# shiveshkhaitan/novel_view_synthesis_3d

Measured on NVIDIA B200. Metric: xunet_train_images_per_sec, higher is better.
Workload: dtype bf16

## Files before the change

novel_view_synthesis_3d_b200/csrc/attn_tc.cu:

```cuda
#include "kernels.h"
#include "tc_common.cuh"

namespace {

struct AttnTcParams {
  const bf16* res;
  bf16* out;
  float* lse;
  int L, C, heads, cross;
  float scale_log2;
  float* cstats;
};

constexpr int kQT = 128;
constexpr int kKB = 64;

__host__ __device__ constexpr int fwd_kv_stages(int hd) { return hd <= 32 ? 6 : 3; }
template <int HD>
__global__ void __launch_bounds__(192) attn_fwd_tc_kernel(const __grid_constant__ CUtensorMap tmQ128,
                                                          const __grid_constant__ CUtensorMap tmKV64, const AttnTcParams p) {
  constexpr int CW = HD < 64 ? HD : 64;
  constexpr int NCH = HD / CW;
  constexpr int TILE = 128 * CW * 2;
  constexpr int TILE_B = kKB * CW * 2;
  constexpr int KV_STAGES = fwd_kv_stages(HD);
  constexpr int P_BYTES = 128 * kKB * 2;
  constexpr int S_BUFS = 2;
  constexpr uint32_t TMEM_COLS = 256;
  constexpr int O_COL = S_BUFS * kKB;
  extern __shared__ uint8_t smem_raw[];
  uint8_t* base = reinterpret_cast<uint8_t*>((reinterpret_cast<uintptr_t>(smem_raw) + 1023) & ~(uintptr_t)1023);
  uint8_t* smQ = base;
  uint8_t* smK = smQ + NCH * TILE;
  uint8_t* smV = smK + KV_STAGES * NCH * TILE_B;
  uint8_t* smP = smV + KV_STAGES * NCH * TILE_B;
  uint64_t* bars = reinterpret_cast<uint64_t*>(smP + 2 * P_BYTES);
  uint64_t* q_full = bars;
  uint64_t* kv_full = bars + 1;
  uint64_t* kv_empty = kv_full + KV_STAGES;
  uint64_t* s_full = kv_empty + KV_STAGES;
  uint64_t* p_full = s_full + 2;
  uint64_t* o_full = p_full + 2;
  uint64_t* o_free = o_full + 1;
  uint32_t* tmem_slot = reinterpret_cast<uint32_t*>(o_free + 1);

  const int warp = threadIdx.x >> 5, lane = threadIdx.x & 31;
  const int q0 = blockIdx.x * kQT, h = blockIdx.y, n = blockIdx.z;
  const int nkv = p.cross ? (n ^ 1) : n;
  const int nkb = p.L / kKB;

  if (threadIdx.x == 0) {
    mbar_init(q_full, 1);
    for (int s = 0; s < KV_STAGES; ++s) { mbar_init(&kv_full[s], 1); mbar_init(&kv_empty[s], 1); }
    for (int s = 0; s < 2; ++s) { mbar_init(&s_full[s], 1); mbar_init(&p_full[s], 128); }
    mbar_init(o_full, 1);
    mbar_init(o_free, 128);
    asm volatile("fence.mbarrier_init.release.cluster;" ::: "memory");
    asm volatile("prefetch.tensormap [%0];" ::"l"(&tmQ128) : "memory");
    asm volatile("prefetch.tensormap [%0];" ::"l"(&tmKV64) : "memory");
  }
  if (warp == 1) tmem_alloc(tmem_slot, TMEM_COLS);
  tcgen05_fence_before();
  __syncthreads();
  tcgen05_fence_after();
  xu_grid_dep_sync();
  const uint32_t tmem_base = *tmem_slot;
  const uint32_t tmem_O = tmem_base + O_COL;

  if (warp == 0) {
    if (lane == 0) {
      mbar_expect_tx(q_full, NCH * TILE);
      for (int c = 0; c < NCH; ++c) tma_load_3d(smQ + c * TILE, &tmQ128, q_full, h * HD + c * CW, q0, n);
      for (int j = 0; j < nkb; ++j) {
        const int s = j % KV_STAGES;
        mbar_wait(&kv_empty[s], ((j / KV_STAGES) & 1) ^ 1);
        mbar_expect_tx(&kv_full[s], 2 * NCH * TILE_B);
        for (int c = 0; c < NCH; ++c) {
          tma_load_3d(smK + (s * NCH + c) * TILE_B, &tmKV64, &kv_full[s], p.C + h * HD + c * CW, j * kKB, nkv);
          tma_load_3d(smV + (s * NCH + c) * TILE_B, &tmKV64, &kv_full[s], 2 * p.C + h * HD + c * CW, j * kKB, nkv);
        }
      }
    }
  } else if (warp == 1) {
    if (lane == 0) {
      const uint32_t idesc_s = make_idesc_bf16(kKB, 0, 0);
      const uint32_t idesc_o = make_idesc_bf16(HD, 0, 1);
      auto issue_s = [&](int j) {
        const int s = j % KV_STAGES;
        mbar_wait(&kv_full[s], (j / KV_STAGES) & 1);
        tcgen05_fence_after();
#pragma unroll
        for (int c = 0; c < NCH; ++c)
#pragma unroll
          for (int k = 0; k < CW / 16; ++k)
            umma_bf16(tmem_base + (j % S_BUFS) * kKB, make_kmajor_desc<CW>(smem_u32(smQ + c * TILE) + k * 32),
                      make_kmajor_desc<CW>(smem_u32(smK + (s * NCH + c) * TILE_B) + k * 32), idesc_s, (c > 0 || k > 0) ? 1u : 0u);
        umma_commit(&s_full[j & 1]);
      };
      mbar_wait(q_full, 0);
      issue_s(0);
      for (int j = 0; j < nkb; ++j) {
        const int s = j % KV_STAGES;
        if (S_BUFS == 2 && j + 1 < nkb) issue_s(j + 1);
        mbar_wait(&p_full[j & 1], (j >> 1) & 1);
        if (S_BUFS == 1 && j + 1 < nkb) issue_s(j + 1);
        if (j > 0) mbar_wait(o_free, (j - 1) & 1);
        tcgen05_fence_after();
#pragma unroll
        for (int kk = 0; kk < kKB / 16; ++kk) {
          const uint64_t dp = make_kmajor_desc<64>(smem_u32(smP + (j & 1) * P_BYTES) + kk * 32);
          const uint64_t dv = make_mnmajor_desc<CW>(smem_u32(smV + s * NCH * TILE_B) + kk * 16 * (CW * 2), TILE_B);
          umma_bf16(tmem_O, dp, dv, idesc_o, kk > 0 ? 1u : 0u);
        }
        umma_commit(o_full);
        umma_commit(&kv_empty[s]);
      }
    }
  } else {
    const int lane_base = (warp & 3) * 32;
    const int r = lane_base + lane;
    const uint32_t lane_addr = (uint32_t)lane_base << 16;
    float m = -INFINITY, l = 0.f, corr_prev = 0.f;
    float acc[HD];
#pragma unroll
    for (int i = 0; i < HD; ++i) acc[i] = 0.f;
    const uint32_t prow_off = (r >> 3) * 1024 + (r & 7) * 128;
    auto absorb_o = [&](int jj, float corr) {
      mbar_wait(o_full, jj & 1);
      tcgen05_fence_after();
#pragma unroll
      for (int c0 = 0; c0 < HD; c0 += 16) {
        uint32_t v[16];
        asm volatile(
            "tcgen05.ld.sync.aligned.32x32b.x16.b32 {%0, %1, %2, %3, %4, %5, %6, %7, %8, %9, %10, %11, %12, %13, %14, %15}, [%16];"
            : "=r"(v[0]), "=r"(v[1]), "=r"(v[2]), "=r"(v[3]), "=r"(v[4]), "=r"(v[5]), "=r"(v[6]), "=r"(v[7]), "=r"(v[8]),
              "=r"(v[9]), "=r"(v[10]), "=r"(v[11]), "=r"(v[12]), "=r"(v[13]), "=r"(v[14]), "=r"(v[15])
            : "r"(tmem_O + lane_addr + c0));
        asm volatile("tcgen05.wait::ld.sync.aligned;" ::: "memory");
#pragma unroll
        for (int i = 0; i < 16; ++i) acc[c0 + i] = fmaf(acc[c0 + i], corr, __uint_as_float(v[i]));
      }
      tcgen05_fence_before();
      mbar_arrive(o_free);
    };
    for (int j = 0; j < nkb; ++j) {
      mbar_wait(&s_full[j & 1], (j >> 1) & 1);
      tcgen05_fence_after();
      uint32_t v[2][32];
      tmem_ld32_nowait(tmem_base + (j % S_BUFS) * kKB + lane_addr, v[0]);
      tmem_ld32_nowait(tmem_base + (j % S_BUFS) * kKB + lane_addr + 32, v[1]);
      asm volatile("tcgen05.wait::ld.sync.aligned;" ::: "memory");
      float mq[4] = {-INFINITY, -INFINITY, -INFINITY, -INFINITY};
#pragma unroll
      for (int i = 0; i < 32; i += 4)
#pragma unroll
        for (int c = 0; c < 4; ++c) mq[c] = fmaxf(mq[c], fmaxf(__uint_as_float(v[0][i + c]), __uint_as_float(v[1][i + c])));
      const float mraw = fmaxf(fmaxf(mq[0], mq[1]), fmaxf(mq[2], mq[3]));
      const float mx = fmaxf(m, mraw * p.scale_log2);
      const float corr = ex2_approx(m - mx);
      float rsq[4] = {0.f, 0.f, 0.f, 0.f};
      uint8_t* prow = smP + (j & 1) * P_BYTES + prow_off;
#pragma unroll
      for (int hh = 0; hh < 2; ++hh)
#pragma unroll
        for (int g = 0; g < 4; ++g) {
          uint4 pk;
          uint32_t* pw = reinterpret_cast<uint32_t*>(&pk);
#pragma unroll
          for (int q = 0; q < 4; ++q) {
            const float p0 = ex2_approx(fmaf(__uint_as_float(v[hh][g * 8 + 2 * q]), p.scale_log2, -mx));
            const float p1 = ex2_approx(fmaf(__uint_as_float(v[hh][g * 8 + 2 * q + 1]), p.scale_log2, -mx));
            rsq[q] += p0 + p1;
            __nv_bfloat162 b2 = __floats2bfloat162_rn(p0, p1);
            pw[q] = *reinterpret_cast<uint32_t*>(&b2);
          }
          const int chunk = hh * 4 + g;
          sts128(prow + ((chunk ^ (r & 7)) << 4), pk);
        }
      l = l * corr + ((rsq[0] + rsq[1]) + (rsq[2] + rsq[3]));
      m = mx;
      fence_async_smem();
      tcgen05_fence_before();
      mbar_arrive(&p_full[j & 1]);
      if (j > 0) absorb_o(j - 1, corr_prev);
      corr_prev = corr;
    }
    absorb_o(nkb - 1, corr_prev);
    const float inv = 1.f / l;
    const long long o = ((long long)n * p.L + q0 + r) * p.C + h * HD;
    float* cs_row = p.cstats ? p.cstats + ((long long)(n >> 1) * p.C + h * HD) * 2 : nullptr;
    float sx[32];
#pragma unroll
    for (int c0 = 0; c0 < HD; c0 += 8) {
      uint4 rv = *reinterpret_cast<const uint4*>(p.res + o + c0);
      const __nv_bfloat162* r2 = reinterpret_cast<const __nv_bfloat162*>(&rv);
      uint4 ov;
// ... 32 lines not shown
};

constexpr int kBB = 64;

__device__ __forceinline__ void bulk_load_1d(void* dst, const void* src, uint32_t bytes, uint64_t* bar) {
  asm volatile("cp.async.bulk.shared::cluster.global.mbarrier::complete_tx::bytes [%0], [%1], %2, [%3];" ::"r"(smem_u32(dst)),
               "l"(src), "r"(bytes), "r"(smem_u32(bar))
               : "memory");
}
__device__ __forceinline__ void tmem_ld16(uint32_t taddr, uint32_t (&v)[16]) {
  asm volatile(
      "tcgen05.ld.sync.aligned.32x32b.x16.b32 {%0, %1, %2, %3, %4, %5, %6, %7, %8, %9, %10, %11, %12, %13, %14, %15}, [%16];"
      : "=r"(v[0]), "=r"(v[1]), "=r"(v[2]), "=r"(v[3]), "=r"(v[4]), "=r"(v[5]), "=r"(v[6]), "=r"(v[7]), "=r"(v[8]), "=r"(v[9]),
        "=r"(v[10]), "=r"(v[11]), "=r"(v[12]), "=r"(v[13]), "=r"(v[14]), "=r"(v[15])
      : "r"(taddr));
  asm volatile("tcgen05.wait::ld.sync.aligned;" ::: "memory");
}

__device__ __forceinline__ void tmem_ld8(uint32_t taddr, uint32_t (&v)[8]) {
  asm volatile("tcgen05.ld.sync.aligned.32x32b.x8.b32 {%0, %1, %2, %3, %4, %5, %6, %7}, [%8];"
               : "=r"(v[0]), "=r"(v[1]), "=r"(v[2]), "=r"(v[3]), "=r"(v[4]), "=r"(v[5]), "=r"(v[6]), "=r"(v[7])
               : "r"(taddr));
  asm volatile("tcgen05.wait::ld.sync.aligned;" ::: "memory");
}

template <int HD>
__global__ void __launch_bounds__(320) attn_bwd_dq_tc_kernel(const __grid_constant__ CUtensorMap tmQ128,
                                                             const __grid_constant__ CUtensorMap tmQ64,
                                                             const __grid_constant__ CUtensorMap tmG128,
                                                             const AttnBwdParams p) {
  constexpr int CW = HD < 64 ? HD : 64;
  constexpr int NCH = HD / CW;
  constexpr int TILE = 128 * CW * 2;
  constexpr int TILE_B = kBB * CW * 2;
  constexpr int STAGES = 2;
  constexpr uint32_t TMEM_COLS = (2 * kBB + HD) <= 256 ? 256 : 512;
  extern __shared__ uint8_t smem_raw[];
// ... 337 lines not shown
#pragma unroll
      for (int q = 0; q < 8; ++q) a2[q] = __floats2bfloat162_rn(__uint_as_float(a[2 * q]) * sc, __uint_as_float(a[2 * q + 1]) * sc);
      *reinterpret_cast<uint4*>(dst + cc) = oa[0];
      *reinterpret_cast<uint4*>(dst + cc + 8) = oa[1];
    }
  }
  tcgen05_fence_before();
  __syncthreads();
  if (warp == 1) {
    tcgen05_fence_after();
    tmem_dealloc(tmem_base, TMEM_COLS);
  }
}

__host__ __device__ constexpr int fused_stages(int hd) { return hd <= 16 ? 4 : 3; }
template <int HD>
__global__ void __launch_bounds__(320, 2) attn_bwd_fused_tc_kernel(const __grid_constant__ CUtensorMap tmQ128,
                                                              const __grid_constant__ CUtensorMap tmQ64,
                                                              const __grid_constant__ CUtensorMap tmG64,
                                                              const __grid_constant__ CUtensorMap tmO64,
                                                              const __grid_constant__ CUtensorMap tmR64,
                                                              const AttnBwdParams p) {
  constexpr int CW = HD < 64 ? HD : 64;
  constexpr int NCH = HD / CW;
  constexpr int TILE = 128 * CW * 2;
  constexpr int TILE_B = kBB * CW * 2;
  constexpr int STAGES = fused_stages(HD);
  constexpr uint32_t TMEM_COLS = 256;
  static_assert(2 * kBB + 4 * HD <= 256, "fused backward: head_dim <= 32");
  extern __shared__ uint8_t smem_raw[];
  uint8_t* base = reinterpret_cast<uint8_t*>((reinterpret_cast<uintptr_t>(smem_raw) + 1023) & ~(uintptr_t)1023);
  uint8_t* smK = base;
  uint8_t* smV = smK + NCH * TILE;
  uint8_t* smQ = smV + NCH * TILE;
  uint8_t* smG = smQ + STAGES * NCH * TILE_B;
  uint8_t* smPT = smG + STAGES * NCH * TILE_B;
  float* smL = reinterpret_cast<float*>(smPT + 2 * 32768);
  float* smD = smL + STAGES * kBB;
  float* smW = smD + STAGES * kBB;
  uint8_t* smO = reinterpret_cast<uint8_t*>(smW + 8 * 64);
  uint8_t* smR = smO + (p.fold ? STAGES * NCH * TILE_B : 0);
  uint64_t* bars = reinterpret_cast<uint64_t*>(smR + (p.fold ? STAGES * NCH * TILE_B : 0));
  uint64_t* kv_full = bars;
  uint64_t* q_full = bars + 1;
  uint64_t* q_empty = q_full + STAGES;
  uint64_t* sp_full = q_empty + STAGES;
  uint64_t* pt_full = sp_full + 1;
  uint64_t* dkv_full = pt_full + 1;
  uint64_t* s_free = dkv_full + 1;
  uint64_t* pt_empty = s_free + 1;
  uint32_t* tmem_slot = reinterpret_cast<uint32_t*>(pt_empty + 2);

// ... 6 lines not shown
    for (int s = 0; s < STAGES; ++s) { mbar_init(&q_full[s], 1); mbar_init(&q_empty[s], 1); }
    mbar_init(sp_full, 1);
    mbar_init(pt_full, 256);
    mbar_init(dkv_full, 1);
    mbar_init(s_free, 256);
    mbar_init(&pt_empty[0], 1); mbar_init(&pt_empty[1], 1);
    asm volatile("fence.mbarrier_init.release.cluster;" ::: "memory");
  }
  if (warp == 1) tmem_alloc(tmem_slot, TMEM_COLS);
  tcgen05_fence_before();
  __syncthreads();
  tcgen05_fence_after();
  xu_grid_dep_sync();
  const uint32_t tmem_base = *tmem_slot;
  const uint32_t tmem_S = tmem_base, tmem_dP = tmem_base + kBB, tmem_dK = tmem_base + 2 * kBB, tmem_dV = tmem_dK + HD, tmem_dQ = tmem_dV + HD;
  const long long lrow = ((long long)nq * p.heads + h) * p.L;

  if (warp == 0) {
    if (lane == 0) {
      mbar_expect_tx(kv_full, 2 * NCH * TILE);
      for (int c = 0; c < NCH; ++c) {
        tma_load_3d(smK + c * TILE, &tmQ128, kv_full, p.C + h * HD + c * CW, k0, mfr);
        tma_load_3d(smV + c * TILE, &tmQ128, kv_full, 2 * p.C + h * HD + c * CW, k0, mfr);
      }
      for (int i = 0; i < nb; ++i) {
        const int s = i % STAGES;
        mbar_wait(&q_empty[s], ((i / STAGES) & 1) ^ 1);
        mbar_expect_tx(&q_full[s], p.fold ? 4 * NCH * TILE_B + kBB * 4 : 2 * NCH * TILE_B + 2 * kBB * 4);
        for (int c = 0; c < NCH; ++c) {
          tma_load_3d(smQ + (s * NCH + c) * TILE_B, &tmQ64, &q_full[s], h * HD + c * CW, i * kBB, nq);
          tma_load_3d(smG + (s * NCH + c) * TILE_B, &tmG64, &q_full[s], h * HD + c * CW, i * kBB, nq);
          if (p.fold) {
            tma_load_3d(smO + (s * NCH + c) * TILE_B, &tmO64, &q_full[s], h * HD + c * CW, i * kBB, nq);
            tma_load_3d(smR + (s * NCH + c) * TILE_B, &tmR64, &q_full[s], h * HD + c * CW, i * kBB, nq);
          }
        }
        bulk_load_1d(smL + s * kBB, p.lse + lrow + i * kBB, kBB * 4, &q_full[s]);
        if (!p.fold) bulk_load_1d(smD + s * kBB, p.Dbuf + lrow + i * kBB, kBB * 4, &q_full[s]);
      }
    }
  } else if (warp == 1) {
    if (lane == 0) {
      const uint32_t idesc_s = make_idesc_bf16(kBB, 0, 0);
      const uint32_t idesc_o = make_idesc_bf16(HD, 0, 1);
      const uint32_t idesc_dq = make_idesc_bf16(HD, 1, 1);
      mbar_wait(kv_full, 0);
      auto issue_scores = [&](int blk) {
        const int s = blk % STAGES;
        mbar_wait(&q_full[s], (blk / STAGES) & 1);
        tcgen05_fence_after();
#pragma unroll
        for (int c = 0; c < NCH; ++c)
#pragma unroll
          for (int k = 0; k < CW / 16; ++k) {
            const uint32_t acc = (c > 0 || k > 0) ? 1u : 0u;
            umma_bf16(tmem_S, make_kmajor_desc<CW>(smem_u32(smK + c * TILE) + k * 32),
                      make_kmajor_desc<CW>(smem_u32(smQ + (s * NCH + c) * TILE_B) + k * 32), idesc_s, acc);
            umma_bf16(tmem_dP, make_kmajor_desc<CW>(smem_u32(smV + c * TILE) + k * 32),
                      make_kmajor_desc<CW>(smem_u32(smG + (s * NCH + c) * TILE_B) + k * 32), idesc_s, acc);
          }
        umma_commit(sp_full);
      };
      issue_scores(0);
      for (int i = 0; i < nb; ++i) {
        const int s = i % STAGES;
        if (i + 1 < nb) {
          mbar_wait(s_free, i & 1);
          issue_scores(i + 1);
        }
        mbar_wait(pt_full, i & 1);
        tcgen05_fence_after();
        const uint32_t pt = smem_u32(smPT) + (uint32_t)((i & 1) * 32768), st = pt + 16384u;
#pragma unroll
        for (int kk = 0; kk < kBB / 16; ++kk) {
          const uint32_t acc = (i > 0 || kk > 0) ? 1u : 0u;
          umma_bf16(tmem_dV, make_kmajor_desc<64>(pt + kk * 32),
                    make_mnmajor_desc<CW>(smem_u32(smG + s * NCH * TILE_B) + kk * 16 * (CW * 2), TILE_B), idesc_o, acc);
          umma_bf16(tmem_dK, make_kmajor_desc<64>(st + kk * 32),
                    make_mnmajor_desc<CW>(smem_u32(smQ + s * NCH * TILE_B) + kk * 16 * (CW * 2), TILE_B), idesc_o, acc);
        }
#pragma unroll
        for (int kk = 0; kk < 128 / 16; ++kk)
          umma_bf16(tmem_dQ + (uint32_t)((i & 1) * HD), make_mnmajor_desc<64>(pt + kk * 16 * 128, 16384),
                    make_mnmajor_desc<CW>(smem_u32(smK) + kk * 16 * (CW * 2), TILE), idesc_dq, kk > 0 ? 1u : 0u);
        umma_commit(&q_empty[s]);
        umma_commit(&pt_empty[i & 1]);
      }
      umma_commit(dkv_full);
    }
  } else {
    const int lane_base = (warp & 3) * 32;
    const int wg = (warp - 2) >> 2;
    const int r = lane_base + lane;
    const uint32_t lane_addr = (uint32_t)lane_base << 16;
    uint8_t* prow0 = smPT + (r >> 3) * 1024 + (r & 7) * 128;
    const int c0 = wg * 32;
    auto flush_dq = [&](int blk) {
      constexpr int HC = HD / 2;
      float* dst = p.dq32 + ((long long)nq * p.L + blk * kBB + (r - 64)) * p.C + h * HD + wg * HC;
      uint32_t v[HC];
      const uint32_t src = tmem_dQ + (uint32_t)((blk & 1) * HD) + lane_addr + wg * HC;
      if constexpr (HC == 8) tmem_ld8(src, v);
      else tmem_ld16(src, v);
#pragma unroll
      for (int j = 0; j < HC; j += 4)
        asm volatile("red.global.add.v4.f32 [%0], {%1, %2, %3, %4};" ::"l"(dst + j), "f"(__uint_as_float(v[j])),
                     "f"(__uint_as_float(v[j + 1])), "f"(__uint_as_float(v[j + 2])), "f"(__uint_as_float(v[j + 3]))
                     : "memory");
    };
    float* wrow = smW + (warp - 2) * 64;
    const uint32_t wrow_a = smem_u32(wrow);
    const float c1 = XU_RSQRT2 * p.scale;
    for (int i = 0; i < nb; ++i) {
      const int s = i % STAGES;
      mbar_wait(&q_full[s], (i / STAGES) & 1);
      if (p.fold) {
        if (wg == 0 && r < kBB) {
          float D = 0.f;
#pragma unroll
          for (int c = 0; c < NCH; ++c)
#pragma unroll
            for (int j = 0; j < CW / 8; ++j) {
              const uint32_t off = (uint32_t)((s * NCH + c) * TILE_B + r * (CW * 2) + j * 16);
// ... 3 lines not shown
              const __nv_bfloat162* g2 = reinterpret_cast<const __nv_bfloat162*>(&gv);
              const __nv_bfloat162* o2 = reinterpret_cast<const __nv_bfloat162*>(&ov);
              const __nv_bfloat162* r2 = reinterpret_cast<const __nv_bfloat162*>(&rv);
#pragma unroll
              for (int q = 0; q < 4; ++q) {
                D = fmaf(__low2float(g2[q]) * XU_RSQRT2, __low2float(o2[q]) * XU_SQRT2 - __low2float(r2[q]), D);
                D = fmaf(__high2float(g2[q]) * XU_RSQRT2, __high2float(o2[q]) * XU_SQRT2 - __high2float(r2[q]), D);
              }
            }
          smD[s * kBB + r] = D;
        }
        named_bar_sync(2, 256);
      }
      mbar_wait(sp_full, i & 1);
      tcgen05_fence_after();
      uint8_t* prow = prow0 + (i & 1) * 32768;
      uint8_t* srow = prow + 16384;
      {
        uint32_t sv[32], dv[32];
        tmem_ld32_nowait(tmem_S + lane_addr + c0, sv);
        tmem_ld32_nowait(tmem_dP + lane_addr + c0, dv);
        __syncwarp();
        sts_f32(wrow + lane, lds_f32(smL + s * kBB + c0 + lane) * -1.4426950408889634f);
        sts_f32(wrow + 32 + lane, lds_f32(smD + s * kBB + c0 + lane) * -p.scale);
        __syncwarp();
        asm volatile("tcgen05.wait::ld.sync.aligned;" ::: "memory");
        tcgen05_fence_before();
        mbar_arrive(s_free);
        mbar_wait(&pt_empty[i & 1], ((i >> 1) & 1) ^ 1);
#pragma unroll
        for (int g = 0; g < 4; ++g) {
          uint4 pk, sk;
          uint32_t* pw = reinterpret_cast<uint32_t*>(&pk);
          uint32_t* sw = reinterpret_cast<uint32_t*>(&sk);
#pragma unroll
          for (int q = 0; q < 4; ++q) {
            const int i0 = g * 8 + 2 * q;
            float2 nl, nd;
            asm volatile("ld.shared.v2.f32 {%0, %1}, [%2];" : "=f"(nl.x), "=f"(nl.y) : "r"(wrow_a + (uint32_t)(i0 * 4)));
            asm volatile("ld.shared.v2.f32 {%0, %1}, [%2];" : "=f"(nd.x), "=f"(nd.y) : "r"(wrow_a + (uint32_t)(128 + i0 * 4)));
            const float p0 = ex2_approx(fmaf(__uint_as_float(sv[i0]), p.scale_log2, nl.x));
            const float p1 = ex2_approx(fmaf(__uint_as_float(sv[i0 + 1]), p.scale_log2, nl.y));
            const float d0 = p0 * fmaf(__uint_as_float(dv[i0]), c1, nd.x);
            const float d1 = p1 * fmaf(__uint_as_float(dv[i0 + 1]), c1, nd.y);
            __nv_bfloat162 a2 = __floats2bfloat162_rn(p0, p1);
            __nv_bfloat162 b2 = __floats2bfloat162_rn(d0, d1);
            pw[q] = *reinterpret_cast<uint32_t*>(&a2);
            sw[q] = *reinterpret_cast<uint32_t*>(&b2);
          }
          const int chunk = (c0 >> 3) + g;
          sts128(prow + ((chunk ^ (r & 7)) << 4), pk);
          sts128(srow + ((chunk ^ (r & 7)) << 4), sk);
        }
      }
      fence_async_smem();
      tcgen05_fence_before();
      mbar_arrive(pt_full);
      if (i > 0 && r >= 64) {
        mbar_wait(&pt_empty[(i - 1) & 1], ((i - 1) >> 1) & 1);
        tcgen05_fence_after();
        flush_dq(i - 1);
      }
    }
    mbar_wait(dkv_full, 0);
    tcgen05_fence_after();
    if (r >= 64) flush_dq(nb - 1);
    bf16* dst = p.dqkv + ((long long)mfr * p.L + k0 + r) * (3LL * p.C) + p.C + h * HD + (wg ? p.C : 0);
    const uint32_t tsrc = wg ? tmem_dV : tmem_dK;
    const float sc = wg ? XU_RSQRT2 : 1.f;
#pragma unroll
    for (int cc = 0; cc < HD; cc += 16) {
      uint32_t a[16];
      tmem_ld16(tsrc + lane_addr + cc, a);
      uint4 oa[2];
      __nv_bfloat162* a2 = reinterpret_cast<__nv_bfloat162*>(oa);
#pragma unroll
      for (int q = 0; q < 8; ++q) a2[q] = __floats2bfloat162_rn(__uint_as_float(a[2 * q]) * sc, __uint_as_float(a[2 * q + 1]) * sc);
      *reinterpret_cast<uint4*>(dst + cc) = oa[0];
      *reinterpret_cast<uint4*>(dst + cc + 8) = oa[1];
    }
    if (p.fold) {
// ... 92 lines not shown
  uint32_t b128[3] = {(uint32_t)CW, 128u, 1u}, b64[3] = {(uint32_t)CW, (uint32_t)kBB, 1u};
  if (!xu_encode_bf16_map(&q128, a.qkv, 3, qd, qs, b128, CW) || !xu_encode_bf16_map(&q64, a.qkv, 3, qd, qs, b64, CW) ||
      !xu_encode_bf16_map(&g128, a.dout, 3, gd, gs, b128, CW) || !xu_encode_bf16_map(&g64, a.dout, 3, gd, gs, b64, CW) ||
      !xu_encode_bf16_map(&o64, a.out, 3, gd, gs, b64, CW) || !xu_encode_bf16_map(&r64, a.res, 3, gd, gs, b64, CW))
    return;
  AttnBwdParams p;
  p.res = (const bf16*)a.res; p.out = (const bf16*)a.out; p.dout = (const bf16*)a.dout;
  p.lse = a.lse; p.Dbuf = a.dscratch; p.dqkv = (bf16*)a.dqkv;
  p.dq32 = a.dscratch + (long long)a.N * a.heads * a.L;
  p.L = a.L; p.C = a.C; p.heads = a.heads; p.cross = a.cross;
  p.scale = 1.f / sqrtf((float)HD);
  p.scale_log2 = 1.4426950408889634f * p.scale;
  p.fold = 0;
  const size_t smem_dq = (size_t)2 * NCH * TILE + 4 * NCH * TILE_B + 16384 + 1024 + 128;
  const size_t smem_dkv = (size_t)2 * NCH * TILE + 4 * NCH * TILE_B + 2 * 16384 + 4 * kBB * 4 + 8 * 64 * 4 + 1024 + 128;
  const size_t smem_fused = (size_t)2 * NCH * TILE + 2 * fused_stages(HD) * NCH * TILE_B + 4 * 16384 + 2 * fused_stages(HD) * kBB * 4 + 8 * 64 * 4 + 1024 + 256;
  static bool configured = false;
  if (!configured) {
    cudaFuncSetAttribute(attn_bwd_dq_tc_kernel<HD>, cudaFuncAttributeMaxDynamicSharedMemorySize, (int)(200 * 1024));
    cudaFuncSetAttribute(attn_bwd_dkv_tc_kernel<HD>, cudaFuncAttributeMaxDynamicSharedMemorySize, (int)(200 * 1024));
    configured = true;
  }
  dim3 grid(a.L / 128, a.heads, a.N);
  if constexpr (HD <= 32) {
    static const bool split = getenv("XUNET_ATTN_BWD_SPLIT") != nullptr;
    if (!split) {
      static bool configured_f = false;
      if (!configured_f) {
        cudaFuncSetAttribute(attn_bwd_fused_tc_kernel<HD>, cudaFuncAttributeMaxDynamicSharedMemorySize, (int)(200 * 1024));
        configured_f = true;
      }
// ... 17 lines not shown
void launch_fwd(const AttnArgs& a, cudaStream_t s) {
  constexpr int CW = HD < 64 ? HD : 64;
  constexpr int NCH = HD / CW;
  constexpr int TILE = 128 * CW * 2;
  constexpr int TILE_B = kKB * CW * 2;
  CUtensorMap tq, tkv;
  uint64_t dims[3] = {(uint64_t)(3 * a.C), (uint64_t)a.L, (uint64_t)a.N};
  uint64_t strides[2] = {(uint64_t)3 * a.C * 2, (uint64_t)a.L * 3 * a.C * 2};
  uint32_t box_q[3] = {(uint32_t)CW, 128u, 1u}, box_kv[3] = {(uint32_t)CW, (uint32_t)kKB, 1u};
  if (!xu_encode_bf16_map(&tq, a.qkv, 3, dims, strides, box_q, CW) || !xu_encode_bf16_map(&tkv, a.qkv, 3, dims, strides, box_kv, CW)) return;
  AttnTcParams p;
  p.res = (const bf16*)a.res; p.out = (bf16*)a.out; p.lse = a.lse;
  p.L = a.L; p.C = a.C; p.heads = a.heads; p.cross = a.cross;
  p.scale_log2 = 1.4426950408889634f / sqrtf((float)HD);
  p.cstats = a.cstats;
  const size_t smem = (size_t)NCH * TILE + 2 * fwd_kv_stages(HD) * NCH * TILE_B + 2 * 128 * kKB * 2 + 1024 + 256;
  static bool configured = false;
  if (!configured) {
    cudaFuncSetAttribute(attn_fwd_tc_kernel<HD>, cudaFuncAttributeMaxDynamicSharedMemorySize, (int)(200 * 1024));
    configured = true;
  }
  dim3 grid(a.L / kQT, a.heads, a.N);
  xu_launch(attn_fwd_tc_kernel<HD>, grid, 192, smem, s, tq, tkv, p);
}

}

bool attn_tc_supported(int dtype, int L, int C, int heads) {
  if (dtype != XU_BF16 || heads <= 0 || C % heads) return false;
  const int hd = C / heads;
  if (hd != 16 && hd != 32 && hd != 64 && hd != 128) return false;
// ... 23 lines not shown
```

novel_view_synthesis_3d_b200/csrc/tc_common.cuh:

```cuda
#pragma once
#include "common.cuh"
#include <cuda.h>

__device__ __forceinline__ uint32_t smem_u32(const void* p) { return (uint32_t)__cvta_generic_to_shared(p); }

__device__ __forceinline__ void mbar_init(uint64_t* bar, uint32_t count) {
  asm volatile("mbarrier.init.shared::cta.b64 [%0], %1;" ::"r"(smem_u32(bar)), "r"(count));
}
__device__ __forceinline__ void mbar_expect_tx(uint64_t* bar, uint32_t bytes) {
  asm volatile("mbarrier.arrive.expect_tx.shared::cta.b64 _, [%0], %1;" ::"r"(smem_u32(bar)), "r"(bytes) : "memory");
}
__device__ __forceinline__ void mbar_wait(uint64_t* bar, uint32_t parity) {
  asm volatile(
      "{\n\t"
      ".reg .pred P1;\n\t"
      "WAIT_LOOP:\n\t"
      "mbarrier.try_wait.parity.shared::cta.b64 P1, [%0], %1;\n\t"
      "@P1 bra DONE;\n\t"
      "bra WAIT_LOOP;\n\t"
      "DONE:\n\t"
      "}" ::"r"(smem_u32(bar)), "r"(parity)
      : "memory");
}
__device__ __forceinline__ void tma_load_4d(void* dst, const CUtensorMap* map, uint64_t* bar, int c0, int c1, int c2, int c3) {
// ... 28 lines not shown
__device__ __forceinline__ void named_bar_sync(int id, int nthreads) { asm volatile("bar.sync %0, %1;" ::"r"(id), "r"(nthreads) : "memory"); }
__device__ __forceinline__ void tcgen05_fence_before() { asm volatile("tcgen05.fence::before_thread_sync;" ::: "memory"); }
__device__ __forceinline__ void tcgen05_fence_after() { asm volatile("tcgen05.fence::after_thread_sync;" ::: "memory"); }
__device__ __forceinline__ void umma_commit(uint64_t* bar) {
  asm volatile("tcgen05.commit.cta_group::1.mbarrier::arrive::one.shared::cluster.b64 [%0];" ::"r"(smem_u32(bar)) : "memory");
}
__device__ __forceinline__ void umma_bf16(uint32_t tmem_d, uint64_t desc_a, uint64_t desc_b, uint32_t idesc, uint32_t accumulate) {
  asm volatile(
      "{\n\t"
      ".reg .pred p;\n\t"
      "setp.ne.b32 p, %4, 0;\n\t"
      "tcgen05.mma.cta_group::1.kind::f16 [%0], %1, %2, %3, p;\n\t"
      "}\n" ::"r"(tmem_d), "l"(desc_a), "l"(desc_b), "r"(idesc), "r"(accumulate)
      : "memory");
}
__device__ __forceinline__ void tmem_ld32(uint32_t taddr, uint32_t (&r)[32]) {
  asm volatile(
      "tcgen05.ld.sync.aligned.32x32b.x32.b32 {%0, %1, %2, %3, %4, %5, %6, %7, %8, %9, %10, %11, %12, %13, %14, %15, %16, %17, "
      "%18, %19, %20, %21, %22, %23, %24, %25, %26, %27, %28, %29, %30, %31}, [%32];"
      : "=r"(r[0]), "=r"(r[1]), "=r"(r[2]), "=r"(r[3]), "=r"(r[4]), "=r"(r[5]), "=r"(r[6]), "=r"(r[7]), "=r"(r[8]), "=r"(r[9]),
        "=r"(r[10]), "=r"(r[11]), "=r"(r[12]), "=r"(r[13]), "=r"(r[14]), "=r"(r[15]), "=r"(r[16]), "=r"(r[17]), "=r"(r[18]),
        "=r"(r[19]), "=r"(r[20]), "=r"(r[21]), "=r"(r[22]), "=r"(r[23]), "=r"(r[24]), "=r"(r[25]), "=r"(r[26]), "=r"(r[27]),
        "=r"(r[28]), "=r"(r[29]), "=r"(r[30]), "=r"(r[31])
      : "r"(taddr));
  asm volatile("tcgen05.wait::ld.sync.aligned;" ::: "memory");
}

__device__ __forceinline__ void tmem_ld32_nowait(uint32_t taddr, uint32_t (&r)[32]) {
  asm volatile(
      "tcgen05.ld.sync.aligned.32x32b.x32.b32 {%0, %1, %2, %3, %4, %5, %6, %7, %8, %9, %10, %11, %12, %13, %14, %15, %16, %17, "
// ... 32 lines not shown
}
__device__ __forceinline__ void sts_f32(void* smem_ptr, float v) {
  asm volatile("st.shared.f32 [%0], %1;" ::"r"(smem_u32(smem_ptr)), "f"(v) : "memory");
}
__device__ __forceinline__ void mbar_arrive(uint64_t* bar) {
  asm volatile("mbarrier.arrive.shared::cta.b64 _, [%0];" ::"r"(smem_u32(bar)) : "memory");
}
__device__ __forceinline__ void fence_async_smem() { asm volatile("fence.proxy.async.shared::cta;" ::: "memory"); }
__device__ __forceinline__ void tmem_alloc(uint32_t* slot, uint32_t ncols) {
  asm volatile("tcgen05.alloc.cta_group::1.sync.aligned.shared::cta.b32 [%0], %1;" ::"r"(smem_u32(slot)), "r"(ncols) : "memory");
  asm volatile("tcgen05.relinquish_alloc_permit.cta_group::1.sync.aligned;" ::: "memory");
}
__device__ __forceinline__ void tmem_dealloc(uint32_t base, uint32_t ncols) {
  asm volatile("tcgen05.dealloc.cta_group::1.sync.aligned.b32 %0, %1;" ::"r"(base), "r"(ncols) : "memory");
}
__device__ __forceinline__ uint32_t make_idesc_bf16(int N, int a_mn_major, int b_mn_major) {
  return (1u << 4) | (1u << 7) | (1u << 10) | ((uint32_t)a_mn_major << 15) | ((uint32_t)b_mn_major << 16) |
         ((uint32_t)(N >> 3) << 17) | ((128u >> 4) << 24);
}

__device__ __forceinline__ float ex2_approx(float x) {
  float y;
  asm("ex2.approx.ftz.f32 %0, %1;" : "=f"(y) : "f"(x));
  return y;
}

template <int S>
__device__ __forceinline__ void xu_wtr_step(float (&x)[32], int lane) {
  const bool up = (lane & S) != 0;
#pragma unroll
  for (int i = 0; i < S; ++i) {
    const float send = up ? x[i] : x[i + S];
    const float keep = up ? x[i + S] : x[i];
// ... 19 lines not shown
```

Before: 2282.

## Keep softmax P in TMEM for attention forward and fused backward MMAs

The forward attention kernel now writes the bf16 probabilities P back into the TMEM columns that held S and feeds them to the PV MMA as a TMEM A operand, instead of staging P through swizzled shared memory. The MMA warp now waits for the previous O MMA before overwriting the next S buffer. The fused backward kernel optionally keeps P^T in TMEM as well (when TMEM columns allow), moves the dQ MMA to use the dS tile with M=64, and restructures the dQ flush to use one warpgroup. This aims to cut shared-memory traffic and footprint, at the cost of extra TMEM store waits and tighter MMA serialization.

New measurement: 2307, median of 6. 1.01x the previous value.

```diff
diff --git a/novel_view_synthesis_3d_b200/csrc/attn_tc.cu b/novel_view_synthesis_3d_b200/csrc/attn_tc.cu
--- a/novel_view_synthesis_3d_b200/csrc/attn_tc.cu
+++ b/novel_view_synthesis_3d_b200/csrc/attn_tc.cu
@@ -13,28 +13,28 @@
 };
 
 constexpr int kQT = 128;
+
 constexpr int kKB = 64;
-
 __host__ __device__ constexpr int fwd_kv_stages(int hd) { return hd <= 32 ? 6 : 3; }
+
 template <int HD>
 __global__ void __launch_bounds__(192) attn_fwd_tc_kernel(const __grid_constant__ CUtensorMap tmQ128,
-                                                          const __grid_constant__ CUtensorMap tmKV64, const AttnTcParams p) {
+                                                          const __grid_constant__ CUtensorMap tmKV, const AttnTcParams p) {
   constexpr int CW = HD < 64 ? HD : 64;
   constexpr int NCH = HD / CW;
   constexpr int TILE = 128 * CW * 2;
-  constexpr int TILE_B = kKB * CW * 2;
+  constexpr int KB = kKB;
+  constexpr int TILE_B = KB * CW * 2;
   constexpr int KV_STAGES = fwd_kv_stages(HD);
-  constexpr int P_BYTES = 128 * kKB * 2;
-  constexpr int S_BUFS = 2;
   constexpr uint32_t TMEM_COLS = 256;
-  constexpr int O_COL = S_BUFS * kKB;
+  constexpr int O_COL = 2 * KB;
+  static_assert(O_COL + HD <= (int)TMEM_COLS, "attn fwd: TMEM layout");
   extern __shared__ uint8_t smem_raw[];
   uint8_t* base = reinterpret_cast<uint8_t*>((reinterpret_cast<uintptr_t>(smem_raw) + 1023) & ~(uintptr_t)1023);
   uint8_t* smQ = base;
   uint8_t* smK = smQ + NCH * TILE;
   uint8_t* smV = smK + KV_STAGES * NCH * TILE_B;
-  uint8_t* smP = smV + KV_STAGES * NCH * TILE_B;
-  uint64_t* bars = reinterpret_cast<uint64_t*>(smP + 2 * P_BYTES);
+  uint64_t* bars = reinterpret_cast<uint64_t*>(smV + KV_STAGES * NCH * TILE_B);
   uint64_t* q_full = bars;
   uint64_t* kv_full = bars + 1;
   uint64_t* kv_empty = kv_full + KV_STAGES;
@@ -47,7 +47,7 @@
   const int warp = threadIdx.x >> 5, lane = threadIdx.x & 31;
   const int q0 = blockIdx.x * kQT, h = blockIdx.y, n = blockIdx.z;
   const int nkv = p.cross ? (n ^ 1) : n;
-  const int nkb = p.L / kKB;
+  const int nkb = p.L / KB;
 
   if (threadIdx.x == 0) {
     mbar_init(q_full, 1);
@@ -57,7 +57,7 @@
     mbar_init(o_free, 128);
     asm volatile("fence.mbarrier_init.release.cluster;" ::: "memory");
     asm volatile("prefetch.tensormap [%0];" ::"l"(&tmQ128) : "memory");
-    asm volatile("prefetch.tensormap [%0];" ::"l"(&tmKV64) : "memory");
+    asm volatile("prefetch.tensormap [%0];" ::"l"(&tmKV) : "memory");
   }
   if (warp == 1) tmem_alloc(tmem_slot, TMEM_COLS);
   tcgen05_fence_before();
@@ -76,14 +76,14 @@
         mbar_wait(&kv_empty[s], ((j / KV_STAGES) & 1) ^ 1);
         mbar_expect_tx(&kv_full[s], 2 * NCH * TILE_B);
         for (int c = 0; c < NCH; ++c) {
-          tma_load_3d(smK + (s * NCH + c) * TILE_B, &tmKV64, &kv_full[s], p.C + h * HD + c * CW, j * kKB, nkv);
-          tma_load_3d(smV + (s * NCH + c) * TILE_B, &tmKV64, &kv_full[s], 2 * p.C + h * HD + c * CW, j * kKB, nkv);
+          tma_load_3d(smK + (s * NCH + c) * TILE_B, &tmKV, &kv_full[s], p.C + h * HD + c * CW, j * KB, nkv);
+          tma_load_3d(smV + (s * NCH + c) * TILE_B, &tmKV, &kv_full[s], 2 * p.C + h * HD + c * CW, j * KB, nkv);
         }
       }
     }
   } else if (warp == 1) {
     if (lane == 0) {
-      const uint32_t idesc_s = make_idesc_bf16(kKB, 0, 0);
+      const uint32_t idesc_s = make_idesc_bf16(KB, 0, 0);
       const uint32_t idesc_o = make_idesc_bf16(HD, 0, 1);
       auto issue_s = [&](int j) {
         const int s = j % KV_STAGES;
@@ -93,7 +93,7 @@
         for (int c = 0; c < NCH; ++c)
 #pragma unroll
           for (int k = 0; k < CW / 16; ++k)
-            umma_bf16(tmem_base + (j % S_BUFS) * kKB, make_kmajor_desc<CW>(smem_u32(smQ + c * TILE) + k * 32),
+            umma_bf16(tmem_base + (j & 1) * KB, make_kmajor_desc<CW>(smem_u32(smQ + c * TILE) + k * 32),
                       make_kmajor_desc<CW>(smem_u32(smK + (s * NCH + c) * TILE_B) + k * 32), idesc_s, (c > 0 || k > 0) ? 1u : 0u);
         umma_commit(&s_full[j & 1]);
       };
@@ -101,16 +101,20 @@
       issue_s(0);
       for (int j = 0; j < nkb; ++j) {
         const int s = j % KV_STAGES;
-        if (S_BUFS == 2 && j + 1 < nkb) issue_s(j + 1);
+        if (j + 1 < nkb) {
+          if (j > 0) {
+            mbar_wait(o_full, (j - 1) & 1);
+            tcgen05_fence_after();
+          }
+          issue_s(j + 1);
+        }
         mbar_wait(&p_full[j & 1], (j >> 1) & 1);
-        if (S_BUFS == 1 && j + 1 < nkb) issue_s(j + 1);
         if (j > 0) mbar_wait(o_free, (j - 1) & 1);
         tcgen05_fence_after();
 #pragma unroll
-        for (int kk = 0; kk < kKB / 16; ++kk) {
-          const uint64_t dp = make_kmajor_desc<64>(smem_u32(smP + (j & 1) * P_BYTES) + kk * 32);
+        for (int kk = 0; kk < KB / 16; ++kk) {
           const uint64_t dv = make_mnmajor_desc<CW>(smem_u32(smV + s * NCH * TILE_B) + kk * 16 * (CW * 2), TILE_B);
-          umma_bf16(tmem_O, dp, dv, idesc_o, kk > 0 ? 1u : 0u);
+          umma_bf16_tmem_a(tmem_O, tmem_base + (j & 1) * KB + kk * 8, dv, idesc_o, kk > 0 ? 1u : 0u);
         }
         umma_commit(o_full);
         umma_commit(&kv_empty[s]);
@@ -124,7 +128,6 @@
     float acc[HD];
 #pragma unroll
     for (int i = 0; i < HD; ++i) acc[i] = 0.f;
-    const uint32_t prow_off = (r >> 3) * 1024 + (r & 7) * 128;
     auto absorb_o = [&](int jj, float corr) {
       mbar_wait(o_full, jj & 1);
       tcgen05_fence_after();
@@ -146,40 +149,38 @@
     for (int j = 0; j < nkb; ++j) {
       mbar_wait(&s_full[j & 1], (j >> 1) & 1);
       tcgen05_fence_after();
-      uint32_t v[2][32];
-      tmem_ld32_nowait(tmem_base + (j % S_BUFS) * kKB + lane_addr, v[0]);
-      tmem_ld32_nowait(tmem_base + (j % S_BUFS) * kKB + lane_addr + 32, v[1]);
+      const uint32_t tS = tmem_base + (j & 1) * KB + lane_addr;
+      uint32_t v[KB / 32][32];
+#pragma unroll
+      for (int hh = 0; hh < KB / 32; ++hh) tmem_ld32_nowait(tS + hh * 32, v[hh]);
       asm volatile("tcgen05.wait::ld.sync.aligned;" ::: "memory");
       float mq[4] = {-INFINITY, -INFINITY, -INFINITY, -INFINITY};
 #pragma unroll
-      for (int i = 0; i < 32; i += 4)
-#pragma unroll
-        for (int c = 0; c < 4; ++c) mq[c] = fmaxf(mq[c], fmaxf(__uint_as_float(v[0][i + c]), __uint_as_float(v[1][i + c])));
+      for (int hh = 0; hh < KB / 32; ++hh)
+#pragma unroll
+        for (int i = 0; i < 32; i += 4)
+#pragma unroll
+          for (int c = 0; c < 4; ++c) mq[c] = fmaxf(mq[c], __uint_as_float(v[hh][i + c]));
       const float mraw = fmaxf(fmaxf(mq[0], mq[1]), fmaxf(mq[2], mq[3]));
       const float mx = fmaxf(m, mraw * p.scale_log2);
       const float corr = ex2_approx(m - mx);
       float rsq[4] = {0.f, 0.f, 0.f, 0.f};
-      uint8_t* prow = smP + (j & 1) * P_BYTES + prow_off;
-#pragma unroll
-      for (int hh = 0; hh < 2; ++hh)
-#pragma unroll
-        for (int g = 0; g < 4; ++g) {
-          uint4 pk;
-          uint32_t* pw = reinterpret_cast<uint32_t*>(&pk);
-#pragma unroll
-          for (int q = 0; q < 4; ++q) {
-            const float p0 = ex2_approx(fmaf(__uint_as_float(v[hh][g * 8 + 2 * q]), p.scale_log2, -mx));
-            const float p1 = ex2_approx(fmaf(__uint_as_float(v[hh][g * 8 + 2 * q + 1]), p.scale_log2, -mx));
-            rsq[q] += p0 + p1;
-            __nv_bfloat162 b2 = __floats2bfloat162_rn(p0, p1);
-            pw[q] = *reinterpret_cast<uint32_t*>(&b2);
-          }
-          const int chunk = hh * 4 + g;
-          sts128(prow + ((chunk ^ (r & 7)) << 4), pk);
-        }
+#pragma unroll
+      for (int hh = 0; hh < KB / 32; ++hh) {
+        uint32_t pk[16];
+#pragma unroll
+        for (int q = 0; q < 16; ++q) {
+          const float p0 = ex2_approx(fmaf(__uint_as_float(v[hh][2 * q]), p.scale_log2, -mx));
+          const float p1 = ex2_approx(fmaf(__uint_as_float(v[hh][2 * q + 1]), p.scale_log2, -mx));
+          rsq[q & 3] += p0 + p1;
+          __nv_bfloat162 b2 = __floats2bfloat162_rn(p0, p1);
+          pk[q] = *reinterpret_cast<uint32_t*>(&b2);
+        }
+        tmem_st16_nowait(tS + hh * 16, pk);
+      }
       l = l * corr + ((rsq[0] + rsq[1]) + (rsq[2] + rsq[3]));
       m = mx;
-      fence_async_smem();
+      tmem_wait_st();
       tcgen05_fence_before();
       mbar_arrive(&p_full[j & 1]);
       if (j > 0) absorb_o(j - 1, corr_prev);
@@ -242,13 +243,6 @@
       : "=r"(v[0]), "=r"(v[1]), "=r"(v[2]), "=r"(v[3]), "=r"(v[4]), "=r"(v[5]), "=r"(v[6]), "=r"(v[7]), "=r"(v[8]), "=r"(v[9]),
         "=r"(v[10]), "=r"(v[11]), "=r"(v[12]), "=r"(v[13]), "=r"(v[14]), "=r"(v[15])
       : "r"(taddr));
-  asm volatile("tcgen05.wait::ld.sync.aligned;" ::: "memory");
-}
-
-__device__ __forceinline__ void tmem_ld8(uint32_t taddr, uint32_t (&v)[8]) {
-  asm volatile("tcgen05.ld.sync.aligned.32x32b.x8.b32 {%0, %1, %2, %3, %4, %5, %6, %7}, [%8];"
-               : "=r"(v[0]), "=r"(v[1]), "=r"(v[2]), "=r"(v[3]), "=r"(v[4]), "=r"(v[5]), "=r"(v[6]), "=r"(v[7])
-               : "r"(taddr));
   asm volatile("tcgen05.wait::ld.sync.aligned;" ::: "memory");
 }
 
@@ -616,6 +610,7 @@
 }
 
 __host__ __device__ constexpr int fused_stages(int hd) { return hd <= 16 ? 4 : 3; }
+__host__ __device__ constexpr bool fused_pt_in_tmem(int hd) { return 2 * kBB + 4 * hd + kBB <= 256; }
 template <int HD>
 __global__ void __launch_bounds__(320, 2) attn_bwd_fused_tc_kernel(const __grid_constant__ CUtensorMap tmQ128,
                                                               const __grid_constant__ CUtensorMap tmQ64,
@@ -628,6 +623,7 @@
   constexpr int TILE = 128 * CW * 2;
   constexpr int TILE_B = kBB * CW * 2;
   constexpr int STAGES = fused_stages(HD);
+  constexpr bool PT_TMEM = fused_pt_in_tmem(HD);
   constexpr uint32_t TMEM_COLS = 256;
   static_assert(2 * kBB + 4 * HD <= 256, "fused backward: head_dim <= 32");
   extern __shared__ uint8_t smem_raw[];
@@ -636,8 +632,9 @@
   uint8_t* smV = smK + NCH * TILE;
   uint8_t* smQ = smV + NCH * TILE;
   uint8_t* smG = smQ + STAGES * NCH * TILE_B;
-  uint8_t* smPT = smG + STAGES * NCH * TILE_B;
-  float* smL = reinterpret_cast<float*>(smPT + 2 * 32768);
+  uint8_t* smST = smG + STAGES * NCH * TILE_B;
+  uint8_t* smPT = smST + 2 * 16384;
+  float* smL = reinterpret_cast<float*>(smPT + (PT_TMEM ? 0 : 2 * 16384));
   float* smD = smL + STAGES * kBB;
   float* smW = smD + STAGES * kBB;
   uint8_t* smO = reinterpret_cast<uint8_t*>(smW + 8 * 64);
@@ -674,6 +671,7 @@
   xu_grid_dep_sync();
   const uint32_t tmem_base = *tmem_slot;
   const uint32_t tmem_S = tmem_base, tmem_dP = tmem_base + kBB, tmem_dK = tmem_base + 2 * kBB, tmem_dV = tmem_dK + HD, tmem_dQ = tmem_dV + HD;
+  const uint32_t tmem_PT = tmem_dQ + 2 * HD;
   const long long lrow = ((long long)nq * p.heads + h) * p.L;
 
   if (warp == 0) {
@@ -703,7 +701,7 @@
     if (lane == 0) {
       const uint32_t idesc_s = make_idesc_bf16(kBB, 0, 0);
       const uint32_t idesc_o = make_idesc_bf16(HD, 0, 1);
-      const uint32_t idesc_dq = make_idesc_bf16(HD, 1, 1);
+      const uint32_t idesc_dq = make_idesc_bf16(HD, 1, 1, 64);
       mbar_wait(kv_full, 0);
       auto issue_scores = [&](int blk) {
         const int s = blk % STAGES;
@@ -730,18 +728,19 @@
         }
         mbar_wait(pt_full, i & 1);
         tcgen05_fence_after();
-        const uint32_t pt = smem_u32(smPT) + (uint32_t)((i & 1) * 32768), st = pt + 16384u;
+        const uint32_t pt = smem_u32(smPT) + (uint32_t)((i & 1) * 16384), st = smem_u32(smST) + (uint32_t)((i & 1) * 16384);
 #pragma unroll
         for (int kk = 0; kk < kBB / 16; ++kk) {
           const uint32_t acc = (i > 0 || kk > 0) ? 1u : 0u;
-          umma_bf16(tmem_dV, make_kmajor_desc<64>(pt + kk * 32),
-                    make_mnmajor_desc<CW>(smem_u32(smG + s * NCH * TILE_B) + kk * 16 * (CW * 2), TILE_B), idesc_o, acc);
+          const uint64_t dg = make_mnmajor_desc<CW>(smem_u32(smG + s * NCH * TILE_B) + kk * 16 * (CW * 2), TILE_B);
+          if constexpr (PT_TMEM) umma_bf16_tmem_a(tmem_dV, tmem_PT + (uint32_t)((i & 1) * 32 + kk * 8), dg, idesc_o, acc);
+          else umma_bf16(tmem_dV, make_kmajor_desc<64>(pt + kk * 32), dg, idesc_o, acc);
           umma_bf16(tmem_dK, make_kmajor_desc<64>(st + kk * 32),
                     make_mnmajor_desc<CW>(smem_u32(smQ + s * NCH * TILE_B) + kk * 16 * (CW * 2), TILE_B), idesc_o, acc);
         }
 #pragma unroll
         for (int kk = 0; kk < 128 / 16; ++kk)
-          umma_bf16(tmem_dQ + (uint32_t)((i & 1) * HD), make_mnmajor_desc<64>(pt + kk * 16 * 128, 16384),
+          umma_bf16(tmem_dQ + (uint32_t)((i & 1) * HD), make_mnmajor_desc<64>(st + kk * 16 * 128, 16384),
                     make_mnmajor_desc<CW>(smem_u32(smK) + kk * 16 * (CW * 2), TILE), idesc_dq, kk > 0 ? 1u : 0u);
         umma_commit(&q_empty[s]);
         umma_commit(&pt_empty[i & 1]);
@@ -753,20 +752,23 @@
     const int wg = (warp - 2) >> 2;
     const int r = lane_base + lane;
     const uint32_t lane_addr = (uint32_t)lane_base << 16;
-    uint8_t* prow0 = smPT + (r >> 3) * 1024 + (r & 7) * 128;
+    const uint32_t row_off = (r >> 3) * 1024 + (r & 7) * 128;
     const int c0 = wg * 32;
+    float* const dq_row = p.dq32 + ((long long)nq * p.L + (warp & 3) * 16 + (lane & 15)) * p.C + h * HD;
     auto flush_dq = [&](int blk) {
-      constexpr int HC = HD / 2;
-      float* dst = p.dq32 + ((long long)nq * p.L + blk * kBB + (r - 64)) * p.C + h * HD + wg * HC;
-      uint32_t v[HC];
-      const uint32_t src = tmem_dQ + (uint32_t)((blk & 1) * HD) + lane_addr + wg * HC;
-      if constexpr (HC == 8) tmem_ld8(src, v);
-      else tmem_ld16(src, v);
-#pragma unroll
-      for (int j = 0; j < HC; j += 4)
-        asm volatile("red.global.add.v4.f32 [%0], {%1, %2, %3, %4};" ::"l"(dst + j), "f"(__uint_as_float(v[j])),
-                     "f"(__uint_as_float(v[j + 1])), "f"(__uint_as_float(v[j + 2])), "f"(__uint_as_float(v[j + 3]))
-                     : "memory");
+      uint32_t v[16];
+#pragma unroll
+      for (int cc = 0; cc < HD; cc += 16) {
+        tmem_ld16(tmem_dQ + (uint32_t)((blk & 1) * HD + cc) + lane_addr, v);
+        if (lane < 16) {
+          float* dst = dq_row + blk * kBB * p.C + cc;
+#pragma unroll
+          for (int j = 0; j < 16; j += 4)
+            asm volatile("red.global.add.v4.f32 [%0], {%1, %2, %3, %4};" ::"l"(dst + j), "f"(__uint_as_float(v[j])),
+                         "f"(__uint_as_float(v[j + 1])), "f"(__uint_as_float(v[j + 2])), "f"(__uint_as_float(v[j + 3]))
+                         : "memory");
+        }
+      }
     };
     float* wrow = smW + (warp - 2) * 64;
     const uint32_t wrow_a = smem_u32(wrow);
@@ -800,8 +802,8 @@
       }
       mbar_wait(sp_full, i & 1);
       tcgen05_fence_after();
-      uint8_t* prow = prow0 + (i & 1) * 32768;
-      uint8_t* srow = prow + 16384;
+      uint8_t* prow = smPT + (i & 1) * 16384 + row_off;
+      uint8_t* srow = smST + (i & 1) * 16384 + row_off;
       {
         uint32_t sv[32], dv[32];
         tmem_ld32_nowait(tmem_S + lane_addr + c0, sv);
@@ -814,6 +816,7 @@
         tcgen05_fence_before();
         mbar_arrive(s_free);
         mbar_wait(&pt_empty[i & 1], ((i >> 1) & 1) ^ 1);
+        if constexpr (PT_TMEM) tcgen05_fence_after();
 #pragma unroll
         for (int g = 0; g < 4; ++g) {
           uint4 pk, sk;
@@ -835,14 +838,16 @@
             sw[q] = *reinterpret_cast<uint32_t*>(&b2);
           }
           const int chunk = (c0 >> 3) + g;
-          sts128(prow + ((chunk ^ (r & 7)) << 4), pk);
+          if constexpr (PT_TMEM) tmem_st4_nowait(tmem_PT + (uint32_t)((i & 1) * 32 + wg * 16 + g * 4) + lane_addr, pw);
+          else sts128(prow + ((chunk ^ (r & 7)) << 4), pk);
           sts128(srow + ((chunk ^ (r & 7)) << 4), sk);
         }
       }
       fence_async_smem();
+      if constexpr (PT_TMEM) tmem_wait_st();
       tcgen05_fence_before();
       mbar_arrive(pt_full);
-      if (i > 0 && r >= 64) {
+      if (i > 0 && wg == 0) {
         mbar_wait(&pt_empty[(i - 1) & 1], ((i - 1) >> 1) & 1);
         tcgen05_fence_after();
         flush_dq(i - 1);
@@ -850,7 +855,7 @@
     }
     mbar_wait(dkv_full, 0);
     tcgen05_fence_after();
-    if (r >= 64) flush_dq(nb - 1);
+    if (wg == 0) flush_dq(nb - 1);
     bf16* dst = p.dqkv + ((long long)mfr * p.L + k0 + r) * (3LL * p.C) + p.C + h * HD + (wg ? p.C : 0);
     const uint32_t tsrc = wg ? tmem_dV : tmem_dK;
     const float sc = wg ? XU_RSQRT2 : 1.f;
@@ -973,7 +978,8 @@
   p.fold = 0;
   const size_t smem_dq = (size_t)2 * NCH * TILE + 4 * NCH * TILE_B + 16384 + 1024 + 128;
   const size_t smem_dkv = (size_t)2 * NCH * TILE + 4 * NCH * TILE_B + 2 * 16384 + 4 * kBB * 4 + 8 * 64 * 4 + 1024 + 128;
-  const size_t smem_fused = (size_t)2 * NCH * TILE + 2 * fused_stages(HD) * NCH * TILE_B + 4 * 16384 + 2 * fused_stages(HD) * kBB * 4 + 8 * 64 * 4 + 1024 + 256;
+  const size_t smem_fused = (size_t)2 * NCH * TILE + 2 * fused_stages(HD) * NCH * TILE_B + (fused_pt_in_tmem(HD) ? 2 : 4) * 16384 +
+                            2 * fused_stages(HD) * kBB * 4 + 8 * 64 * 4 + 1024 + 256;
   static bool configured = false;
   if (!configured) {
     cudaFuncSetAttribute(attn_bwd_dq_tc_kernel<HD>, cudaFuncAttributeMaxDynamicSharedMemorySize, (int)(200 * 1024));
@@ -1021,7 +1027,7 @@
   p.L = a.L; p.C = a.C; p.heads = a.heads; p.cross = a.cross;
   p.scale_log2 = 1.4426950408889634f / sqrtf((float)HD);
   p.cstats = a.cstats;
-  const size_t smem = (size_t)NCH * TILE + 2 * fwd_kv_stages(HD) * NCH * TILE_B + 2 * 128 * kKB * 2 + 1024 + 256;
+  const size_t smem = (size_t)NCH * TILE + 2 * fwd_kv_stages(HD) * NCH * TILE_B + 1024 + 256;
   static bool configured = false;
   if (!configured) {
     cudaFuncSetAttribute(attn_fwd_tc_kernel<HD>, cudaFuncAttributeMaxDynamicSharedMemorySize, (int)(200 * 1024));
diff --git a/novel_view_synthesis_3d_b200/csrc/tc_common.cuh b/novel_view_synthesis_3d_b200/csrc/tc_common.cuh
--- a/novel_view_synthesis_3d_b200/csrc/tc_common.cuh
+++ b/novel_view_synthesis_3d_b200/csrc/tc_common.cuh
@@ -66,6 +66,27 @@
       "}\n" ::"r"(tmem_d), "l"(desc_a), "l"(desc_b), "r"(idesc), "r"(accumulate)
       : "memory");
 }
+__device__ __forceinline__ void umma_bf16_tmem_a(uint32_t tmem_d, uint32_t tmem_a, uint64_t desc_b, uint32_t idesc, uint32_t accumulate) {
+  asm volatile(
+      "{\n\t"
+      ".reg .pred p;\n\t"
+      "setp.ne.b32 p, %4, 0;\n\t"
+      "tcgen05.mma.cta_group::1.kind::f16 [%0], [%1], %2, %3, p;\n\t"
+      "}\n" ::"r"(tmem_d), "r"(tmem_a), "l"(desc_b), "r"(idesc), "r"(accumulate)
+      : "memory");
+}
+__device__ __forceinline__ void tmem_st16_nowait(uint32_t taddr, const uint32_t (&v)[16]) {
+  asm volatile(
+      "tcgen05.st.sync.aligned.32x32b.x16.b32 [%0], {%1, %2, %3, %4, %5, %6, %7, %8, %9, %10, %11, %12, %13, %14, %15, %16};"
+      ::"r"(taddr), "r"(v[0]), "r"(v[1]), "r"(v[2]), "r"(v[3]), "r"(v[4]), "r"(v[5]), "r"(v[6]), "r"(v[7]), "r"(v[8]), "r"(v[9]),
+        "r"(v[10]), "r"(v[11]), "r"(v[12]), "r"(v[13]), "r"(v[14]), "r"(v[15])
+      : "memory");
+}
+__device__ __forceinline__ void tmem_st4_nowait(uint32_t taddr, const uint32_t* v) {
+  asm volatile("tcgen05.st.sync.aligned.32x32b.x4.b32 [%0], {%1, %2, %3, %4};" ::"r"(taddr), "r"(v[0]), "r"(v[1]), "r"(v[2]), "r"(v[3])
+               : "memory");
+}
+__device__ __forceinline__ void tmem_wait_st() { asm volatile("tcgen05.wait::st.sync.aligned;" ::: "memory"); }
 __device__ __forceinline__ void tmem_ld32(uint32_t taddr, uint32_t (&r)[32]) {
   asm volatile(
       "tcgen05.ld.sync.aligned.32x32b.x32.b32 {%0, %1, %2, %3, %4, %5, %6, %7, %8, %9, %10, %11, %12, %13, %14, %15, %16, %17, "
@@ -128,9 +149,9 @@
 __device__ __forceinline__ void tmem_dealloc(uint32_t base, uint32_t ncols) {
   asm volatile("tcgen05.dealloc.cta_group::1.sync.aligned.b32 %0, %1;" ::"r"(base), "r"(ncols) : "memory");
 }
-__device__ __forceinline__ uint32_t make_idesc_bf16(int N, int a_mn_major, int b_mn_major) {
+__device__ __forceinline__ uint32_t make_idesc_bf16(int N, int a_mn_major, int b_mn_major, int M = 128) {
   return (1u << 4) | (1u << 7) | (1u << 10) | ((uint32_t)a_mn_major << 15) | ((uint32_t)b_mn_major << 16) |
-         ((uint32_t)(N >> 3) << 17) | ((128u >> 4) << 24);
+         ((uint32_t)(N >> 3) << 17) | ((uint32_t)(M >> 4) << 24);
 }
 
 __device__ __forceinline__ float ex2_approx(float x) {
```
